# hku-mars/ImMesh

Measured on AMD Instinct MI355X. Metric: scans/sec (reg+mesh), 100k-pt scan into 10M-voxel map, higher is better.
Workload: dtype f64

## Files before the change

immesh_amd/csrc/c_api.cpp:

```cpp
#include "host_ctx.hpp"
#include "imu_host.hpp"
#include <cmath>
#include <new>

#define RP_ABORTED 1
static thread_local std::string g_create_error;
thread_local KProf* g_kprof = nullptr;



extern "C" {

void immesh_default_config(immesh_config* c) {
    std::memset(c, 0, sizeof(*c));
    c->voxel_size = 0.5; c->max_layer = 2;
    for (int i = 0; i < 5; i++) c->layer_init[i] = 5;
    c->max_points_size = 100; c->planer_threshold = 0.01; c->dept_err = 0.02; c->beam_err = 0.05; c->calib_laser = 0;
    c->sigma_num = 3.0; c->max_iter = 4;
    c->extR[0] = c->extR[4] = c->extR[8] = 1.0;
    c->extT[0] = 0.04165; c->extT[1] = 0.02326; c->extT[2] = -0.0284;
    c->mesh_min_spacing = 0.1; c->mesh_voxel = 0.4; c->mesh_region = 10.0; c->mesh_append_budget = 10000;
}

const char* immesh_create_error(void) { return g_create_error.c_str(); }
const char* immesh_last_error(immesh_ctx* c) { return c ? c->err.c_str() : "null ctx"; }

static int alloc_all(immesh_ctx* c) {
    const immesh_config& g = c->cfg;
    RegMapDev& m = c->map;
    const int64_t cap_roots = g.cap_root_voxels > 0 ? g.cap_root_voxels : (1 << 20);
    const int64_t cap_nodes = g.cap_nodes > 0 ? g.cap_nodes : cap_roots + cap_roots / 2;
    const int64_t cap_chunks = g.cap_point_chunks > 0 ? g.cap_point_chunks : cap_nodes * 2;
    const int64_t cap_ext = g.max_points_size > IM_INLINE_CHUNKS * IM_CHUNK_PTS ? std::max<int64_t>(1024, cap_nodes / 4) : std::max<int64_t>(1024, cap_nodes / 64);
    const int64_t hcap = np2(cap_roots * 2);
    if (cap_nodes > 0x7fffffff || cap_chunks > 0x7fffffff || hcap > 0xffffffffLL) { c->err = "capacity too large for 32-bit indices"; return IMMESH_E_INVAL; }
    int rc;
#define A(ptr, n) if ((rc = c->dalloc(&(ptr), (size_t)(n)))) return rc
    A(m.htab, hcap); A(m.slot_head, hcap);
    m.hmask = (uint64_t)hcap - 1;
    A(m.nodes, cap_nodes);
    const int64_t cap_leaf = std::max<int64_t>(4096, cap_nodes / 2);
    A(m.leaf_chunks, cap_leaf * 16); m.cap_leaf_chunks = (int32_t)cap_leaf;
    A(m.chunk_data, cap_chunks * IM_CHUNK_PTS * IM_PT_DOUBLES); A(m.ext_tables, cap_ext * IM_EXT_CHUNKS);
    A(m.counters, 16); A(m.free_ready, cap_chunks); A(m.free_pending, cap_chunks);
    m.cap_nodes = (int32_t)cap_nodes; m.cap_chunks = (int32_t)cap_chunks; m.cap_ext = (int32_t)cap_ext;
    m.max_layer = g.max_layer; m.max_points_size = g.max_points_size;
    for (int i = 0; i < 5; i++) m.init_size[i] = g.layer_init[i];
    m.planer_threshold = (float)g.planer_threshold;
    m.voxel_size_f = (float)g.voxel_size;
    m.voxel_size_d = g.voxel_size;
    m.shard_rank = g.shard_world > 1 ? g.shard_rank : 0; m.shard_world = g.shard_world > 1 ? g.shard_world : 1;
    m.shard_brick_log2 = g.shard_brick_log2 > 0 ? g.shard_brick_log2 : 5;
    m.shard_scheme = g.shard_scheme == 1 ? 1 : 0;
    HIPCHK(c, hipMemsetAsync(m.counters, 0, 16 * sizeof(int32_t), c->stream));
    HIPCHK(c, hipMemsetAsync(m.htab, 0xFF, hcap * sizeof(HashEnt), c->stream));
    HIPCHK(c, hipMemsetAsync(m.slot_head, 0, hcap * sizeof(unsigned long long), c->stream));
    m.upd_seq = 0;
    A(c->d_stats, STATS_WORDS);
    if (c->knobs.debug) { A(c->reg_dbg, REG_DBG_WORDS); HIPCHK(c, hipMemsetAsync(c->reg_dbg, 0, (size_t)REG_DBG_WORDS * 8, c->stream)); }
    HIPCHK(c, hipMemsetAsync(c->d_stats, 0, STATS_WORDS * sizeof(int64_t), c->stream));

    const int64_t ns = g.cap_scan_points > 0 ? g.cap_scan_points : 600000;
    c->cap_scan = ns;
    A(c->d_pts_down, ns * 3); A(c->d_pts_raw, ns * 4);
    A(c->d_partials, ((ns + 63) / 64) * RES_NR); A(c->d_out48, RES_NV); A(c->d_done, 4);
    HIPCHK(c, hipMemsetAsync(c->d_done, 0, 16, c->stream));
    A(c->d_match, ns); A(c->d_mnode, ns); A(c->d_dis, ns); A(c->d_rinv, ns); A(c->d_normal, ns * 3);
    A(c->d_ptdata, ns * IM_PT_DOUBLES);
    A(c->d_key_a, ns); A(c->d_key_b, ns); A(c->d_idx_a, ns); A(c->d_idx_b, ns); A(c->d_idx_c, ns);
    A(c->d_slot, ns); A(c->d_slot_s, ns); A(c->d_seg_start, ns); A(c->d_nseg, 16); A(c->d_ds_out, ns * 3);
    c->sort_temp_bytes = std::max({sort_pairs_u64_temp_bytes((int)ns), sort_pairs_u32_temp_bytes((int)ns), exclusive_sum_temp_bytes((int)ns)}) + 256;
    { char* t; A(t, c->sort_temp_bytes); c->d_sort_temp = t; }
    A(c->p_key_a, ns); A(c->p_key_b, ns); A(c->p_idx_a, ns); A(c->p_idx_b, ns); A(c->p_idx_c, ns); A(c->p_seg, ns); A(c->p_nseg, 16); A(c->p_slot, ns); A(c->p_slot_s, ns); A(c->p_pool4, ns * 4);
    { char* t; A(t, c->sort_temp_bytes); c->p_sort_temp = t; }
    {
        unsigned long long cap = 1024; while (cap < 2ull * (unsigned long long)ns) cap <<= 1;
        char* t; A(t, cap * 16); c->p_htab = t; c->p_htab_cap = cap;
        launch_ds_table_reset(c->stream, t, cap);
        if ((rc = c->pinned(&c->h_ds_dyn, &c->d_ds_dyn, 1)) || (rc = c->pinned(&c->h_ds_info, &c->d_ds_info, 16))) return rc;
        HIPCHK(c, hipMemsetAsync(c->p_nseg, 0, 16 * sizeof(int32_t), c->stream));
    }
    {
        m.split_general = c->knobs.split_general >= 0 ? c->knobs.split_general : (g.max_layer >= 3 ? 1 : 0);
        A(m.sub_order, ns); A(m.sub_items, 2 * ns);
        HIPCHK(c, hipMemsetAsync(m.sub_items, 0, (size_t)2 * ns * sizeof(unsigned long long), c->stream));
    }
    A(c->d_dump_count, 2);
    A(c->d_touched, 2 * ns + 16);
    A(c->d_regstate, 1);
    A(c->d_epi, 8);
    HIPCHK(c, hipMemsetAsync(c->d_epi, 0, 32, c->stream));
    for (int q = 0; q < 2; q++) { A(c->d_rp_slots[q], RP_SLOT_DOUBLES); launch_fill_u64(c->stream, (unsigned long long*)c->d_rp_slots[q], RP_SLOT_SENTINEL, RP_SLOT_DOUBLES); }
    HIPCHK(c, hipMemsetAsync(c->d_regstate, 0, sizeof(RegState), c->stream));
    A(c->d_und_in, ns * 5); A(c->d_und_out, ns * 4); A(c->d_und_tab, 64 * 23 + 24);
#undef A
    if ((rc = c->pinned(&c->h_out48, &c->d_out48_host, RES_NV)) || (rc = c->pinned(&c->h_reg_out, &c->d_reg_out_host, REG_OUT_DOUBLES)) ||
        (rc = c->pinned(&c->h_epi_flag, &c->d_epi_flag_host, 8)) || (rc = c->pinned(&c->h_counters, &c->d_counters_host, 16))) return rc;
    return 0;
}


immesh_ctx* immesh_create(const immesh_config* cfg) {
    g_create_error.clear();
    if (!cfg) { g_create_error = "null config"; return nullptr; }
    int ndev = 0;
    hipError_t e = hipGetDeviceCount(&ndev);
    if (e != hipSuccess || ndev <= 0) {
        g_create_error = std::string("no usable HIP device (") + (e != hipSuccess ? hipGetErrorString(e) : "count 0") + "); the hot path has no CPU fallback";
        return nullptr;
    }
    if (cfg->device < 0 || cfg->device >= ndev) { g_create_error = "device ordinal out of range"; return nullptr; }
    if (cfg->max_layer < 0 || cfg->max_layer > 4 || cfg->voxel_size <= 0 || cfg->max_iter < 1) { g_create_error = "invalid config"; return nullptr; }
    if (cfg->shard_world > 1 && (cfg->shard_rank < 0 || cfg->shard_rank >= cfg->shard_world || cfg->shard_brick_log2 < 0 || cfg->shard_brick_log2 > 16)) { g_create_error = "invalid shard configuration"; return nullptr; }
    immesh_ctx* c = new (std::nothrow) immesh_ctx();
    if (!c) { g_create_error = "out of host memory"; return nullptr; }
    c->cfg = *cfg;
    c->knobs = Knobs::from_env(MESH_NPAR);
    std::memset(&c->cnt, 0, sizeof(c->cnt));
    int prio_greatest = 0;
    if (hipSetDevice(cfg->device) == hipSuccess) (void)hipDeviceGetStreamPriorityRange(&c->prio_least, &prio_greatest);
    if (c->knobs.no_priority) prio_greatest = c->prio_least = 0;
    if (c->knobs.make_stream(&c->stream, prio_greatest, false) != hipSuccess) {
        g_create_error = "hipSetDevice/hipStreamCreate failed"; delete c; return nullptr;
    }
    for (auto& ev : c->ev) (void)hipEventCreate(&ev);
    if (c->knobs.make_stream(&c->stream_pre, 0, true) != hipSuccess || hipEventCreateWithFlags(&c->ev_inputs_free, hipEventDisableTiming) != hipSuccess ||
        hipEventRecord(c->ev_inputs_free, c->stream) != hipSuccess || !(c->ev_inputs_cur = c->ev_inputs_free)) {
        g_create_error = "hipStreamCreate/hipEventCreate failed"; immesh_destroy(c); return nullptr;
    }
    { const double s = std::sin((double)(float)cfg->beam_err * 0.017453293); c->dvar_beam = s * s; }
    { const double s = std::sin((double)(float)0.01 * 0.017453293); c->dvar_calib = s * s; }
    {
        const int resident = residual_persistent_resident_blocks(cfg->device);
        c->rp_max_blocks = c->knobs.rp_blocks ? c->knobs.rp_blocks : std::max(1, resident / 2 - 1);
    }
    int rc = alloc_all(c);
    if (!rc) rc = mesh_alloc(c);
    if (!rc && hipStreamSynchronize(c->stream) != hipSuccess) { rc = IMMESH_E_HIP; c->err = "initialisation kernels failed"; }
    if (rc) { g_create_error = c->err; immesh_destroy(c); return nullptr; }
// ... 645 lines not shown
```

immesh_amd/csrc/reg_kernels.hip:

```cpp
#include <algorithm>
#include <cstdlib>
#include "regmap.hpp"
#include "kernels.hpp"
#include "prof.hpp"

using namespace imd;

struct PlaneRegs { double n[3], c[3], pv[21]; float d, radius; };
struct BestMatch { int node; int layer; double prob; bool ok; PlaneRegs P; };

IMD double plane_sigma(const double* pv, const double* J) {
    double tmp[6];
#pragma unroll
    for (int c = 0; c < 6; c++) {
        double s = 0;
#pragma unroll
        for (int r = 0; r < 6; r++) s += J[r] * pv[(r <= c) ? sym21_index(r, c) : sym21_index(c, r)];
        tmp[c] = s;
    }
    double sig = 0;
#pragma unroll
    for (int c = 0; c < 6; c++) sig += tmp[c] * J[c];
    return sig;
}
// ... 1074 lines not shown
        else v = e < 36 ? rs->p11inv[e] : (e < 108 ? rs->tmat[e - 36] : (e < 132 ? rs->st[e - 108] : (e < 156 ? rs->prior[e - 132] : (e < 160 ? rs->tot[e - 156] : (double)rs->rematch))));
        L[400 + e] = v;
    }
    if (a.it == 0) {
        for (int e = lane; e < 108; e += 64) { if (e < 36) rs->p11inv[e] = a.mat[e]; else rs->tmat[e - 36] = a.mat[e]; }
        if (lane < 24) rs->prior[lane] = a.prior[lane];
        const unsigned long long* src = (const unsigned long long*)&a.sp;
        unsigned long long* dst = (unsigned long long*)&rs->sp;
        for (int e = lane; e < (int)(sizeof(ScanParams) / 8); e += 64) dst[e] = src[e];
    }
    __syncthreads();
    if (lane == 0) { L[400 + 156] += L[64 + RES_PLANE_TESTS]; L[400 + 157] += L[64 + RES_EXTRA_PROBE]; L[400 + 159] += L[64 + RES_N_MATCH]; }
    __syncthreads();
    ekf_step_wave(rs, L + 400, a.mat, L + 64 + RES_HTH, L + 64 + RES_HTZ, L[64 + RES_N_MATCH], L[64 + RES_SUM_DIS], L + 128, lane, a.it, a.max_iter, a.sp.extR, reg_out, ticket);
}

IMD float4 transform_value(const double* extR, const double* extT, const double* R, const double* t, const float4 v) {
    const double p[3] = {(double)v.x, (double)v.y, (double)v.z};
    double pi[3], pw[3];
    m3_vec(extR, p, pi);
    pi[0] += extT[0]; pi[1] += extT[1]; pi[2] += extT[2];
    m3_vec(R, pi, pw);
    return make_float4((float)(pw[0] + t[0]), (float)(pw[1] + t[1]), (float)(pw[2] + t[2]), v.w);
}
IMD void transform_point(const double* extR, const double* extT, const double* R, const double* t, const float4* __restrict__ raw, float4* __restrict__ world, const int i) {
    world[i] = transform_value(extR, extT, R, t, raw[i]);
}
IMD void point_var_point(const RegMapDev& m, const ScanParams& sp, const float* __restrict__ pts, const int i, const int stride, const int mode,
                         double* __restrict__ pt_data, unsigned long long* __restrict__ sort_key, uint32_t* __restrict__ slot_out, int32_t* __restrict__ pt_next,
                         const unsigned long long hint_key, const unsigned int hint_slot, const int hint_root) {
    const double p[3] = {(double)pts[(size_t)i * stride + 0], (double)pts[(size_t)i * stride + 1], (double)pts[(size_t)i * stride + 2]};
    double pimu[3], pwd[3];
    m3_vec(sp.extR, p, pimu);
    pimu[0] += sp.extT[0]; pimu[1] += sp.extT[1]; pimu[2] += sp.extT[2];
    m3_vec(sp.R, pimu, pwd);
    pwd[0] += sp.t[0]; pwd[1] += sp.t[1]; pwd[2] += sp.t[2];
    const double pw[3] = {(double)(float)pwd[0], (double)(float)pwd[1], (double)(float)pwd[2]};
    double bcov[9], cm[9], a[9];
    if (mode == 0) {
        double pz[3] = {p[0], p[1], p[2]};
        if (pz[2] == 0) pz[2] = 0.001;
        calc_body_var(pz, sp.dept_err, sp.dvar_beam, bcov);
        double pimu_z[3];
        m3_vec(sp.extR, pz, pimu_z);
        pimu_z[0] += sp.extT[0]; pimu_z[1] += sp.extT[1]; pimu_z[2] += sp.extT[2];
        skew(pimu_z, cm);
        m3_sandwich(sp.RextR, bcov, a);
    } else {
        double pl[3] = {p[0], p[1], p[2]};
        calc_body_var(pl, sp.dept_err, sp.dvar_beam, bcov);
        skew(pl, cm);
        m3_sandwich(sp.R, bcov, a);
    }
    double nc[9], tmp[9], b[9], var[9];
#pragma unroll
    for (int k = 0; k < 9; k++) nc[k] = -cm[k];
    m3_mul(nc, sp.rot_var, tmp);
    m3_mul_bt(tmp, nc, b);
#pragma unroll
    for (int k = 0; k < 9; k++) var[k] = (a[k] + b[k]) + sp.t_var[k];
    double* o = pt_data + (size_t)i * IM_PT_DOUBLES;
    o[0] = pw[0]; o[1] = pw[1]; o[2] = pw[2];
    o[3] = var[0]; o[4] = var[1]; o[5] = var[2]; o[6] = var[4]; o[7] = var[5]; o[8] = var[8];
    const double key = sqrt(var[0] * var[0] + var[4] * var[4] + var[8] * var[8]);
    sort_key[i] = (unsigned long long)__double_as_longlong(key);
    int64_t kx[3];
#pragma unroll
    for (int j = 0; j < 3; j++) kx[j] = key_axis(pw[j] / (double)m.voxel_size_f);
    const uint64_t pk = pack_key(kx[0], kx[1], kx[2]);
    if (m.shard_world > 1 && !shard_keeps(m, kx[0], kx[1], kx[2])) { slot_out[i] = 0xFFFFFFFFu; return; }
    bool created = false;
    const bool hinted = hint_root >= 0 && pk == hint_key;
    const int64_t slot = hinted ? (int64_t)hint_slot : hash_find_or_insert(m, pk, &created);
    if (slot < 0) { m.counters[5] = 5; slot_out[i] = 0xFFFFFFFFu; return; }
    if (created) {
        const float vs = m.voxel_size_f;
        const double c[3] = {(0.5 + (double)kx[0]) * (double)vs, (0.5 + (double)kx[1]) * (double)vs, (0.5 + (double)kx[2]) * (double)vs};
        const int node = node_alloc(m, 0, c, vs / 4, pk, 0);
        m.htab[slot].root = node;
        atomicAdd(&m.counters[6], 1);
    }
    slot_out[i] = (uint32_t)slot;
    if (pt_next) {
        const unsigned long long mine = ((unsigned long long)(unsigned int)m.upd_seq << 32) | (unsigned int)i;
        const unsigned long long old = atomicExch(&m.slot_head[slot], mine);
        const bool first = (unsigned int)(old >> 32) != (unsigned int)m.upd_seq;
        const unsigned long long fm = __ballot(first);
        if (first) {
            pt_next[i] = -1;
            const int lane = (int)(threadIdx.x & 63), leader = __builtin_ctzll(fm);
            int base = 0;
            if (lane == leader) base = atomicAdd(&m.counters[7], (int)__popcll(fm));
            base = __shfl(base, leader, 64);
            const int k = base + (int)__popcll(fm & ((1ull << lane) - 1ull));
            m.touched[2 * (size_t)k] = (uint32_t)slot; m.touched[2 * (size_t)k + 1] = hinted ? (uint32_t)hint_root : (uint32_t)m.htab[slot].root;
        }
        else pt_next[i] = (int)(unsigned int)(old & 0xFFFFFFFFull);
    }
}

__global__ __launch_bounds__(256) void point_var_kernel(RegMapDev m, ScanParams sp, const ScanParams* __restrict__ spd, const float* __restrict__ pts, int n, int stride, int mode,
                                                         double* __restrict__ pt_data, unsigned long long* __restrict__ sort_key, uint32_t* __restrict__ slot_out,
                                                         int32_t* __restrict__ pt_next, const float4* __restrict__ raw, float4* __restrict__ world, int n_raw, int nb_pv) {
    if ((int)blockIdx.x >= nb_pv) {
        const int i = ((int)blockIdx.x - nb_pv) * 256 + threadIdx.x;
        if (i >= n_raw) return;
        const ScanParams* q = spd ? spd : &sp;
        double R[9], t[3];
#pragma unroll
        for (int k = 0; k < 9; k++) R[k] = q->R[k];
#pragma unroll
        for (int k = 0; k < 3; k++) t[k] = q->t[k];
        transform_point(sp.extR, sp.extT, R, t, raw, world, i);
        return;
    }
    const int i = blockIdx.x * blockDim.x + threadIdx.x;
    if (i >= n) return;
    if (spd) {
#pragma unroll
        for (int k = 0; k < 9; k++) { sp.R[k] = spd->R[k]; sp.RextR[k] = spd->RextR[k]; sp.rot_var[k] = spd->rot_var[k]; sp.t_var[k] = spd->t_var[k]; }
#pragma unroll
        for (int k = 0; k < 3; k++) sp.t[k] = spd->t[k];
    }
    point_var_point(m, sp, pts, i, stride, mode, pt_data, sort_key, slot_out, pt_next);
}

__global__ void segment_heads_kernel(const uint32_t* __restrict__ sorted_slot, int n, int32_t* __restrict__ seg_start, int32_t* __restrict__ nseg) {
    const int i = blockIdx.x * blockDim.x + threadIdx.x;
    if (i >= n) return;
    if (sorted_slot[i] == 0xFFFFFFFFu) return;
    if (i == 0 || sorted_slot[i - 1] != sorted_slot[i]) seg_start[atomicAdd(nseg, 1)] = i;
}

struct WaveCtx { int lane; int64_t* stats; int root; bool shared = false; };

struct PlaneFit { double c[3], ev[3], U[9]; int imin, imax; bool planar; };
IMD double sel3(const int i, const double a, const double b, const double c) { return i == 0 ? a : (i == 1 ? b : c); }

template <class FE>
IMD void fit_eigen(FE&& for_each_point, const int n, const float planer_threshold, PlaneFit& f) {
    double s[9];
#pragma unroll
    for (int k = 0; k < 9; k++) s[k] = 0;
    for_each_point([&](const double* q) __attribute__((always_inline)) {
        const double x = q[0], y = q[1], z = q[2];
        s[0] += x; s[1] += y; s[2] += z;
        s[3] += x * x; s[4] += x * y; s[5] += x * z; s[6] += y * y; s[7] += y * z; s[8] += z * z;
    });
#pragma unroll
    for (int k = 0; k < 9; k++) s[k] = wave_sum_fast(s[k]);
    const double dn = (double)n;
    f.c[0] = s[0] / dn; f.c[1] = s[1] / dn; f.c[2] = s[2] / dn;
    double cov[9];
    cov[0] = s[3] / dn - f.c[0] * f.c[0]; cov[1] = s[4] / dn - f.c[0] * f.c[1]; cov[2] = s[5] / dn - f.c[0] * f.c[2];
    cov[3] = cov[1];                      cov[4] = s[6] / dn - f.c[1] * f.c[1]; cov[5] = s[7] / dn - f.c[1] * f.c[2];
    cov[6] = cov[2];                      cov[7] = cov[5];                      cov[8] = s[8] / dn - f.c[2] * f.c[2];
    sym3_eigen_jacobi_fast(cov, f.ev, f.U);
    const double e0 = f.ev[0], e1 = f.ev[1], e2 = f.ev[2];
    int imin = 0, imax = 0;
    double emin = e0, emax = e0;
    if (e1 < emin) { imin = 1; emin = e1; }
    if (e2 < emin) { imin = 2; emin = e2; }
    if (e1 > emax) { imax = 1; emax = e1; }
    if (e2 > emax) { imax = 2; emax = e2; }
    f.imin = imin; f.imax = imax;
    f.planar = emin < (double)planer_threshold;
}

template <class FE>
IMD void fit_plane_var(FE&& for_each_point, const int n, const PlaneFit& f, double* pv) {
#pragma clang fp contract(fast)
    const int imin = f.imin, m1 = imin == 0 ? 1 : 0, m2 = imin == 2 ? 1 : 2;
    double um1[3], um2[3], umin[3];
#pragma unroll
    for (int r = 0; r < 3; r++) {
        const double u0 = f.U[r * 3 + 0], u1 = f.U[r * 3 + 1], u2 = f.U[r * 3 + 2];
        um1[r] = sel3(m1, u0, u1, u2);
        um2[r] = sel3(m2, u0, u1, u2);
        umin[r] = sel3(imin, u0, u1, u2);
    }
// ... 450 lines not shown
            if (last_refit_n) { (void)wave_init_plane(m, node, last_refit_n, wq); last_refit_n = 0; }
            if (w.lane == 0) { nd.flags = nd.flags & ~NF_UPDATE_EN; node_free_points(m, node); nd.newpts = 0; }
            __builtin_amdgcn_fence(__ATOMIC_RELEASE, "workgroup");
            npts = 0; newp = 0;
            j++;
            if (w.lane == 0 && w.stats && n_ref) { atomicAdd((unsigned long long*)&w.stats[0], (unsigned long long)n_ref); atomicAdd((unsigned long long*)&w.stats[1], (unsigned long long)n_ref_pts); }
            return j;
        }
    }
    write_counts();
    if (last_refit_n) (void)wave_init_plane(m, node, last_refit_n, wq);
    if (w.lane == 0 && w.stats && n_ref) { atomicAdd((unsigned long long*)&w.stats[0], (unsigned long long)n_ref); atomicAdd((unsigned long long*)&w.stats[1], (unsigned long long)n_ref_pts); }
    return j;
}

__global__ __launch_bounds__(256) void replay_kernel(RegMapDev m, const uint32_t* __restrict__ sorted_slot, const int32_t* __restrict__ sorted_idx,
                                                      const double* __restrict__ pt_data, int n, const int32_t* __restrict__ seg_start,
                                                      const int32_t* __restrict__ nseg, int mode, int64_t* stats) {
    __shared__ int stacks[4][48];
    const int wv = threadIdx.x >> 6;
    const int seg = blockIdx.x * 4 + wv;
    if (seg >= *nseg) return;
    WaveCtx w; w.lane = threadIdx.x & 63; w.stats = stats;
    const int start = seg_start[seg];
    const uint32_t slot = sorted_slot[start];
    const int root = m.htab[slot].root;
    if (root < 0) return;
    w.root = root;
    if (mode == 0) {
        for (int j = start; j < n && sorted_slot[j] == slot; j++)
            wave_update_point(m, root, pt_data + (size_t)sorted_idx[j] * IM_PT_DOUBLES, stacks[wv], w);
    } else {
        int cnt = m.nodes[root].npts;
        for (int j = start; j < n && sorted_slot[j] == slot; j++) {
            if (!wave_push_point(m, root, cnt, pt_data + (size_t)sorted_idx[j] * IM_PT_DOUBLES, w)) return;
            cnt++;
        }
        if (w.lane == 0) { m.nodes[root].npts = cnt; m.nodes[root].newpts = cnt; }
        __builtin_amdgcn_fence(__ATOMIC_RELEASE, "workgroup");
        if (cnt > m.init_size[0]) wave_init_octo_tree(m, root, stacks[wv], w);
    }
}

#define RL_CAP 64
#define DBG_FUSED_OFF 64
#define DBG_FUSED_RECS 16384
#define DBG_RES_OFF (DBG_FUSED_OFF + DBG_FUSED_RECS * 8)
static_assert(DBG_RES_OFF + 8 * 512 * 8 == REG_DBG_WORDS, "the IMMESH_DEBUG buffer (kernels.hpp) holds the counters and both trace areas");
#define RF_PTS 128
__global__ __launch_bounds__(256, 3) void replay_fused_kernel(RegMapDev m, const int32_t* __restrict__ pt_next, const unsigned long long* __restrict__ sort_key,
                                                            const double* __restrict__ pt_data, int64_t* stats, uint32_t* __restrict__ general_list,
                                                            unsigned long long* __restrict__ dbg, unsigned long long* flag_dev, unsigned long long* flag_host,
                                                            unsigned long long flag_seq) {
    if (flag_dev && blockIdx.x == 0 && threadIdx.x == 0) {
        __hip_atomic_store(flag_dev, flag_seq, __ATOMIC_RELAXED, __HIP_MEMORY_SCOPE_AGENT);
        __hip_atomic_store(flag_host, flag_seq, __ATOMIC_RELAXED, __HIP_MEMORY_SCOPE_SYSTEM);
    }
    __shared__ unsigned long long skey[4][RL_CAP];
    __shared__ int sidx[4][RL_CAP];
    __shared__ int order[4][RL_CAP];
    __builtin_amdgcn_s_setprio(REG_UPD_PRIO);
    const int wv = threadIdx.x >> 6, lane = threadIdx.x & 63;
    const int t_first = blockIdx.x * 4 + wv, t_stride = gridDim.x * 4;
    uint32_t slot_first = m.touched[2 * (size_t)t_first];
    int root_first = (int)m.touched[2 * (size_t)t_first + 1];
    const int n_touched = m.counters[7];
#define FDBG(k) do { if (dbg) { const unsigned long long _t = __builtin_readcyclecounter(); if (tr) ((unsigned int*)tr)[4 + (k)] = (unsigned int)(_t - tprev); tprev = _t; } } while (0)
#define FEND(state, nref) do { if (tr) { tr[1] = __builtin_amdgcn_s_memrealtime(); tr[7] = (unsigned long long)((unsigned)cnt | ((unsigned)(nref) << 8) | ((unsigned)(state) << 16)); } } while (0)
    auto process = [&](const int t, const uint32_t slot, int root) __attribute__((always_inline)) {
    unsigned long long* const tr = (dbg && lane == 0 && t < DBG_FUSED_RECS) ? dbg + DBG_FUSED_OFF + (size_t)t * 8 : nullptr;
    unsigned long long tprev = dbg ? __builtin_readcyclecounter() : 0;
    if (tr) { tr[0] = __builtin_amdgcn_s_memrealtime(); tr[2] = tr[3] = tr[4] = tr[5] = tr[6] = tr[7] = 0; }
    if (root < 0) root = m.htab[slot].root;
    if (root < 0) return;
    FDBG(0);
    NodeRec& nd = m.nodes[root];
    const int flags = nd.flags, layer = nd.layer;
    const int npts = nd.npts, newp = nd.newpts;
    if (dbg) { asm volatile("s_waitcnt vmcnt(0)" ::: "memory"); FDBG(1); }
    int chunks[IM_INLINE_CHUNKS];
#pragma unroll
    for (int k = 0; k < IM_INLINE_CHUNKS; k++) chunks[k] = nd.chunks[k];
    if (dbg) { asm volatile("s_waitcnt vmcnt(0)" ::: "memory"); FDBG(2); }
    int cnt = 0;
    int ihead = (int)(unsigned int)(m.slot_head[slot] & 0xFFFFFFFFull);
    if (dbg) { asm volatile("s_waitcnt vmcnt(0)" ::: "memory"); FDBG(3); }
    for (int i = ihead; i >= 0; i = pt_next[i]) {
        if (cnt < RL_CAP && lane == 0) { skey[wv][cnt] = sort_key[i]; sidx[wv][cnt] = i; }
        cnt++;
    }
    FDBG(4);
    const int want = NF_INIT | NF_PLANE | NF_UPDATE_EN;
    if (layer == 0 && (flags & want) == (NF_INIT | NF_PLANE)) { FEND(1, 0); return; }
    const int ntot = npts + cnt;
    bool hand_over = cnt > RL_CAP || (flags & want) != want || layer != 0 || newp > 5 || ntot > RF_PTS || ntot >= m.max_points_size;
    if (!hand_over) {
        __builtin_amdgcn_fence(__ATOMIC_RELEASE, "workgroup");
        __builtin_amdgcn_wave_barrier();
        __builtin_amdgcn_fence(__ATOMIC_ACQUIRE, "workgroup");
        for (int e = lane; e < cnt; e += 64) {
            const unsigned long long k = skey[wv][e];
            const int id = sidx[wv][e];
            int rank = 0;
            for (int f = 0; f < cnt; f++) { const unsigned long long kf = skey[wv][f]; rank += (kf < k || (kf == k && sidx[wv][f] < id)) ? 1 : 0; }
            order[wv][rank] = id;
        }
        __builtin_amdgcn_fence(__ATOMIC_RELEASE, "workgroup");
        __builtin_amdgcn_wave_barrier();
        __builtin_amdgcn_fence(__ATOMIC_ACQUIRE, "workgroup");
        FDBG(5);
        auto chunk_of = [&](int ci) { int c = chunks[0];
#pragma unroll
            for (int k = 1; k < IM_INLINE_CHUNKS; k++) { const int ck = chunks[k]; c = (ci == k) ? ck : c; }
            return c; };
        const int n_ref = (newp + cnt) / 6;
        double P0[9], P1[9];
#pragma unroll
        for (int k = 0; k < 9; k++) { P0[k] = 0; P1[k] = 0; }
        {
            const int q0 = lane, q1 = lane + 64;
            const double* s0 = nullptr; const double* s1 = nullptr;
            if (q0 < ntot && (q0 >= npts || n_ref > 0))
                s0 = q0 < npts ? m.chunk_data + ((size_t)chunk_of(q0 >> 4) * IM_CHUNK_PTS + (q0 & 15)) * IM_PT_DOUBLES : pt_data + (size_t)order[wv][q0 - npts] * IM_PT_DOUBLES;
            if (q1 < ntot && (q1 >= npts || n_ref > 0))
                s1 = q1 < npts ? m.chunk_data + ((size_t)chunk_of(q1 >> 4) * IM_CHUNK_PTS + (q1 & 15)) * IM_PT_DOUBLES : pt_data + (size_t)order[wv][q1 - npts] * IM_PT_DOUBLES;
            if (s0) {
#pragma unroll
                for (int k = 0; k < 9; k++) P0[k] = s0[k]; }
            if (s1) {
#pragma unroll
                for (int k = 0; k < 9; k++) P1[k] = s1[k]; }
        }
        if (dbg) asm volatile("s_waitcnt vmcnt(0)" ::: "memory");
        FDBG(6);
        PlaneFit fit;
        long long n_ref_pts = 0;
        int n_last = 0;
        for (int r = 0; r < n_ref && !hand_over; r++) {
            const int nr = npts + 6 * (r + 1) - newp;
            n_ref_pts += nr;
            auto fe = [&](auto&& fn) __attribute__((always_inline)) { if (lane < nr) fn(P0); if (lane + 64 < nr) fn(P1); };
            if (r + 1 < n_ref) {
                double s1[3] = {0, 0, 0}, s2[3] = {0, 0, 0};
                fe([&](const double* q) __attribute__((always_inline)) {
#pragma unroll
                    for (int a = 0; a < 3; a++) { s1[a] += q[a]; s2[a] += q[a] * q[a]; } });
#pragma unroll
                for (int a = 0; a < 3; a++) { s1[a] = wave_sum_fast(s1[a]); s2[a] = wave_sum_fast(s2[a]); }
                const double dn = (double)nr;
                double vmin = 1e300, mag = 0;
#pragma unroll
                for (int a = 0; a < 3; a++) { const double mu = s1[a] / dn; const double v = s2[a] / dn - mu * mu; vmin = fmin(vmin, v); mag += s2[a] / dn; }
                if (vmin + (1e-7 + 1e-12 * mag) < (double)m.planer_threshold) continue;
            }
            fit_eigen(fe, nr, m.planer_threshold, fit);
            if (!fit.planar) hand_over = true;
            n_last = nr;
        }
        FDBG(7);
        if (!hand_over) {
            const int c_first = (npts + IM_CHUNK_PTS - 1) >> 4, c_last = (ntot - 1) >> 4;
            if (cnt > 0 && c_first <= c_last) {
                int c = 0;
                const bool need = lane >= c_first && lane <= c_last && lane < IM_INLINE_CHUNKS && chunk_of(lane) < 0;
                if (need) c = alloc_chunk(m);
                if (__ballot(need && c < 0)) return;
#pragma unroll
                for (int k = 0; k < IM_INLINE_CHUNKS; k++) { const int ck = __shfl(c, k, 64); const int nk = __shfl(need ? 1 : 0, k, 64); if (nk) chunks[k] = ck; }
            }
            {
                const int q0 = lane, q1 = lane + 64;
                if (q0 >= npts && q0 < ntot) { double* d = m.chunk_data + ((size_t)chunk_of(q0 >> 4) * IM_CHUNK_PTS + (q0 & 15)) * IM_PT_DOUBLES;
#pragma unroll
                    for (int k = 0; k < 9; k++) d[k] = P0[k]; }
                if (q1 >= npts && q1 < ntot) { double* d = m.chunk_data + ((size_t)chunk_of(q1 >> 4) * IM_CHUNK_PTS + (q1 & 15)) * IM_PT_DOUBLES;
#pragma unroll
                    for (int k = 0; k < 9; k++) d[k] = P1[k]; }
            }
            if (lane == 0) {
                nd.npts = ntot; nd.newpts = (newp + cnt) % 6;
#pragma unroll
                for (int k = 0; k < IM_INLINE_CHUNKS; k++) nd.chunks[k] = chunks[k];
                if (n_ref) { int64_t* sh = stats + 16 + (size_t)(t & 63) * 16; atomicAdd((unsigned long long*)&sh[0], (unsigned long long)n_ref); atomicAdd((unsigned long long*)&sh[1], (unsigned long long)n_ref_pts); }
            }
            FDBG(8);
            if (n_ref > 0) {
                double pv[21];
                auto fe = [&](auto&& fn) __attribute__((always_inline)) { if (lane < n_last) fn(P0); if (lane + 64 < n_last) fn(P1); };
                fit_plane_var(fe, n_last, fit, pv);
                fit_store(nd, fit, pv, lane);
            }
            FDBG(9);
            FEND(2, n_ref);
            return;
        }
    }
    if (lane == 0) general_list[atomicAdd(&m.counters[10], 1)] = slot;
    FEND(3, 0);
    };
    for (int t = t_first; t < n_touched; t += t_stride) {
        if (t != t_first) { slot_first = m.touched[2 * (size_t)t]; root_first = (int)m.touched[2 * (size_t)t + 1]; }
        process(t, slot_first, root_first);
    }
#undef FDBG
#undef FEND
}

__device__ bool replay_split_root(const RegMapDev& m, const int root, const int* order, const int cnt, const double* __restrict__ pt_data, const WaveCtx& w);
__device__ bool replay_split_leaves(const RegMapDev& m, const int root, const int* order, const int cnt, const double* __restrict__ pt_data, const WaveCtx& w, int* s_key, int* s_first);
__global__ __launch_bounds__(256) void replay_list_kernel(RegMapDev m, const int32_t* __restrict__ pt_next, const unsigned long long* __restrict__ sort_key,
                                                           const double* __restrict__ pt_data, int64_t* stats, int32_t* __restrict__ big_idx, int32_t* __restrict__ big_order,
                                                           unsigned long long* __restrict__ dbg, const uint32_t* __restrict__ work, const int32_t* __restrict__ n_work) {
    __shared__ unsigned long long skey[4][RL_CAP];
    __shared__ int sidx[4][RL_CAP];
    __shared__ int order[4][RL_CAP];
    __shared__ int stacks[4][48];
    __builtin_amdgcn_s_setprio(REG_UPD_PRIO);
    const int wv = threadIdx.x >> 6;
    const int nw = *n_work;
    WaveCtx w; w.lane = threadIdx.x & 63; w.stats = stats;
    for (int t = blockIdx.x * 4 + wv; t < nw; t += gridDim.x * 4) {
        const uint32_t slot = work[t];
        const int root = m.htab[slot].root;
        if (root < 0) continue;
        w.root = root;
        const unsigned long long tdbg0 = dbg ? __builtin_readcyclecounter() : 0;
        __builtin_amdgcn_wave_barrier();
        int cnt = 0;
        for (int i = (int)(unsigned int)(m.slot_head[slot] & 0xFFFFFFFFull); i >= 0; i = pt_next[i]) {
            if (cnt < RL_CAP && w.lane == 0) { skey[wv][cnt] = sort_key[i]; sidx[wv][cnt] = i; }
            cnt++;
        }
        if (cnt > RL_CAP) {
            int base = 0;
            if (w.lane == 0) base = atomicAdd(&m.counters[9], cnt);
            base = __shfl(base, 0, 64);
            if (w.lane == 0) { int k = 0; for (int i = (int)(unsigned int)(m.slot_head[slot] & 0xFFFFFFFFull); i >= 0; i = pt_next[i]) big_idx[base + k++] = i; }
            __builtin_amdgcn_fence(__ATOMIC_RELEASE, "agent");
            __builtin_amdgcn_wave_barrier();
            __builtin_amdgcn_fence(__ATOMIC_ACQUIRE, "agent");
            for (int e = w.lane; e < cnt; e += 64) {
                const int id = big_idx[base + e];
                const unsigned long long k = sort_key[id];
                int rank = 0;
                for (int f = 0; f < cnt; f++) { const int idf = big_idx[base + f]; const unsigned long long kf = sort_key[idf]; rank += (kf < k || (kf == k && idf < id)) ? 1 : 0; }
                big_order[base + rank] = id;
            }
            __builtin_amdgcn_fence(__ATOMIC_RELEASE, "agent");
            __builtin_amdgcn_wave_barrier();
            __builtin_amdgcn_fence(__ATOMIC_ACQUIRE, "agent");
            if (replay_split_root(m, root, big_order + base, cnt, pt_data, w)) continue;
            int jb = wave_replay_planar_root(m, root, big_order + base, cnt, pt_data, w);
            if (jb == 0) jb = wave_replay_planar_node(m, root, big_order + base, cnt, pt_data, w);
            for (int j = jb; j < cnt; j++) wave_update_point(m, root, pt_data + (size_t)big_order[base + j] * IM_PT_DOUBLES, stacks[wv], w);
            continue;
        }
        __builtin_amdgcn_fence(__ATOMIC_RELEASE, "workgroup");
        __builtin_amdgcn_wave_barrier();
        __builtin_amdgcn_fence(__ATOMIC_ACQUIRE, "workgroup");
        for (int e = w.lane; e < cnt; e += 64) {
            const unsigned long long k = skey[wv][e];
            const int id = sidx[wv][e];
            int rank = 0;
            for (int f = 0; f < cnt; f++) { const unsigned long long kf = skey[wv][f]; rank += (kf < k || (kf == k && sidx[wv][f] < id)) ? 1 : 0; }
            order[wv][rank] = id;
        }
        __builtin_amdgcn_fence(__ATOMIC_RELEASE, "workgroup");
        __builtin_amdgcn_wave_barrier();
        __builtin_amdgcn_fence(__ATOMIC_ACQUIRE, "workgroup");
        if (replay_split_leaves(m, root, order[wv], cnt, pt_data, w, (int*)skey[wv], sidx[wv])) continue;
        if (replay_split_root(m, root, order[wv], cnt, pt_data, w)) continue;
        const unsigned long long tdbg1 = dbg ? __builtin_readcyclecounter() : 0;
        int jf = wave_replay_planar_root(m, root, order[wv], cnt, pt_data, w);
        if (jf == 0) jf = wave_replay_planar_node(m, root, order[wv], cnt, pt_data, w);
        for (int j = jf; j < cnt; j++) wave_update_point(m, root, pt_data + (size_t)order[wv][j] * IM_PT_DOUBLES, stacks[wv], w);
        if (dbg && w.lane == 0) {
            const unsigned long long t2 = __builtin_readcyclecounter();
            atomicMax(&dbg[jf == cnt ? 8 : 9], ((t2 - tdbg0) << 16) | (unsigned long long)cnt);
            atomicAdd(&dbg[jf == cnt ? 10 : 11], t2 - tdbg1);
            atomicAdd(&dbg[jf == cnt ? 12 : 13], 1ull);
            atomicAdd(&dbg[14], tdbg1 - tdbg0);
        }
    }
}

#define SPLIT_MISSING 0x40000000
__device__ __noinline__ bool replay_split_leaves(const RegMapDev& m, const int root, const int* order, const int cnt, const double* __restrict__ pt_data, const WaveCtx& w, int* s_key, int* s_first) {
    const NodeRec& nr = m.nodes[root];
    const int flags = nr.flags;
    if (!m.split_general || cnt < 2 || cnt > RL_CAP || !(flags & NF_INIT) || (flags & NF_PLANE) || nr.layer >= m.max_layer || m.cap_nodes >= (1 << 26)) return false;
    if (w.lane == 0 && nr.npts != 0) node_free_points(m, root);
    const int lane = w.lane;
    int key = -1;
    if (lane < cnt) {
        const double* q = pt_data + (size_t)order[lane] * IM_PT_DOUBLES;
        const double qx = q[0], qy = q[1], qz = q[2];
        int nd = root;
        for (int depth = 0; depth < 8; depth++) {
            const NodeRec& r = m.nodes[nd];
            const int f = r.flags, layer = r.layer, npts = r.npts;
            if (!((f & NF_INIT) && !(f & NF_PLANE) && layer < m.max_layer && (npts == 0 || nd == root))) { key = nd; break; }
            const int oct = 4 * (qx > r.center[0] ? 1 : 0) + 2 * (qy > r.center[1] ? 1 : 0) + (qz > r.center[2] ? 1 : 0);
            const int child = r.child[oct];
            if (child < 0) { key = nd | (oct << 26) | SPLIT_MISSING; break; }
            nd = child;
        }
        if (key < 0) key = nd;
    }
    if (lane < cnt) s_key[lane] = key;
    __builtin_amdgcn_fence(__ATOMIC_RELEASE, "workgroup");
    __builtin_amdgcn_wave_barrier();
    __builtin_amdgcn_fence(__ATOMIC_ACQUIRE, "workgroup");
    int first = lane, rank = 0, size = 0;
    if (lane < cnt) {
        first = -1;
        for (int f = 0; f < cnt; f++) {
            const bool same = s_key[f] == key;
            if (same && first < 0) first = f;
            if (same && f < lane) rank++;
            if (same) size++;
        }
        s_first[lane] = first;
    }
    __builtin_amdgcn_fence(__ATOMIC_RELEASE, "workgroup");
    __builtin_amdgcn_wave_barrier();
    __builtin_amdgcn_fence(__ATOMIC_ACQUIRE, "workgroup");
    int before = 0;
    if (lane < cnt) for (int f = 0; f < cnt; f++) before += s_first[f] < first ? 1 : 0;
    const bool leader = lane < cnt && first == lane;
    const unsigned long long lm = __ballot(leader);
    const int n_items = (int)__popcll(lm);
    int seg = 0, item0 = 0;
    if (lane == 0) { seg = atomicAdd(&m.counters[11], cnt); item0 = atomicAdd(&m.counters[12], n_items); }
    seg = __shfl(seg, 0, 64); item0 = __shfl(item0, 0, 64);
    if (lane < cnt) m.sub_order[seg + before + rank] = order[lane];
    if (leader) {
        const int it = item0 + (int)__popcll(lm & ((1ull << lane) - 1ull));
        const int start = (key & SPLIT_MISSING) ? (key & ((1 << 26) - 1)) : key;
        m.sub_items[2 * (size_t)it] = (unsigned long long)(unsigned int)start | ((unsigned long long)(unsigned int)root << 32);
        m.sub_items[2 * (size_t)it + 1] = (unsigned long long)(unsigned int)(seg + before) | ((unsigned long long)(unsigned int)size << 32);
    }
    return true;
}
__device__ bool replay_split_root(const RegMapDev& m, const int root, const int* order, const int cnt, const double* __restrict__ pt_data, const WaveCtx& w) {
    const NodeRec& nr = m.nodes[root];
    const int flags = nr.flags;
    if (!m.split_general || cnt < 8 || !(flags & NF_INIT) || (flags & NF_PLANE) || nr.layer >= m.max_layer) return false;
    if (w.lane == 0 && nr.npts != 0) node_free_points(m, root);
// ... 190 lines not shown
```

immesh_amd/csrc/regmap.hpp:

```cpp
#pragma once
#include "dev_math.hpp"

#define IM_CHUNK_PTS 16
#define IM_PT_DOUBLES 9
#define IM_INLINE_CHUNKS 8
#define IM_EXT_CHUNKS 2048
#define IM_LEAF_SLOTS 15
#define IM_G_MAX_POINTS 1000

#define NF_INIT 1
#define NF_PLANE 2
#define NF_UPDATE_EN 4

struct alignas(64) NodeRec {
    int32_t child[8];
    int32_t flags, layer, npts, newpts;
    float quarter, d, radius, min_eig;
    double center[3];
    double p_center[3];
    double p_normal[3];
    double p_var[21];
    int32_t chunks[IM_INLINE_CHUNKS];
    int32_t ext, path;
    unsigned long long key;
    int32_t leaf_head;
    int32_t lock;
    unsigned long long pad[3];
};
static_assert(sizeof(NodeRec) == 384, "NodeRec layout");

struct HashEnt { unsigned long long key; int32_t root; int32_t pad; };

struct RegMapDev {
    HashEnt* htab;
    uint64_t hmask;
    NodeRec* nodes;
    double* chunk_data;
    int32_t* ext_tables;
    int32_t* counters;
    int32_t* free_ready;
    int32_t* free_pending;
    int32_t* leaf_chunks;
    int32_t cap_leaf_chunks;
    unsigned long long* slot_head;
    uint32_t* touched;
    int32_t split_general;
    int32_t* sub_order;
    unsigned long long* sub_items;
    int32_t upd_seq;
    int32_t shard_rank, shard_world, shard_brick_log2, shard_scheme;
    int32_t cap_nodes, cap_chunks, cap_ext;
    int32_t max_layer, max_points_size, init_size[5];
    float planer_threshold;
    float voxel_size_f;
    double voxel_size_d;
};

namespace imd {

IMD int sym21_index(int r, int c) {
    return r * 6 - (r * (r - 1)) / 2 + (c - r);
}

IMHD int brick_owner(int scheme, int world, int64_t bx, int64_t by, int64_t bz, uint64_t packed) {
    if (scheme == 1 || world % 3 == 0 || world % 5 == 0) return (int)(hash64(packed) % (uint64_t)world);
    const int64_t c = (bx + 3 * by + 5 * bz) % (int64_t)world;
    return (int)(c < 0 ? c + world : c);
}
IMD int shard_owner(const RegMapDev& m, int64_t kx, int64_t ky, int64_t kz) {
    const int b = m.shard_brick_log2;
    return brick_owner(m.shard_scheme, m.shard_world, kx >> b, ky >> b, kz >> b, pack_key(kx >> b, ky >> b, kz >> b));
}
IMD bool shard_keeps(const RegMapDev& m, int64_t kx, int64_t ky, int64_t kz) {
    if (shard_owner(m, kx, ky, kz) == m.shard_rank) return true;
    const int64_t msk = ((int64_t)1 << m.shard_brick_log2) - 1;
    const int64_t lx = kx & msk, ly = ky & msk, lz = kz & msk;
    if (lx != 0 && lx != msk && ly != 0 && ly != msk && lz != 0 && lz != msk) return false;
    for (int dx = -1; dx <= 1; dx++)
        for (int dy = -1; dy <= 1; dy++)
            for (int dz = -1; dz <= 1; dz++)
                if ((dx | dy | dz) != 0 && shard_owner(m, kx + dx, ky + dy, kz + dz) == m.shard_rank) return true;
    return false;
}

IMD int64_t hash_find(const RegMapDev& m, uint64_t key) {
    uint64_t h = hash64(key) & m.hmask;
    for (int probe = 0; probe < 4096; probe++) {
        const unsigned long long k = m.htab[h].key;
        if (k == key) return (int64_t)h;
        if (k == IM_KEY_EMPTY) return -1;
        h = (h + 1) & m.hmask;
    }
    return -1;
}
IMD int64_t hash_find_or_insert(const RegMapDev& m, uint64_t key, bool* created) {
    uint64_t h = hash64(key) & m.hmask;
    *created = false;
    for (int probe = 0; probe < 4096; probe++) {
        unsigned long long k = m.htab[h].key;
        if (k == key) return (int64_t)h;
        if (k == IM_KEY_EMPTY) {
            const unsigned long long prev = atomicCAS(&m.htab[h].key, (unsigned long long)IM_KEY_EMPTY, (unsigned long long)key);
            if (prev == IM_KEY_EMPTY) { *created = true; return (int64_t)h; }
            if (prev == key) return (int64_t)h;
        }
        h = (h + 1) & m.hmask;
    }
    return -1;
}

IMD int alloc_chunk(const RegMapDev& m) {
    if (__hip_atomic_load(&m.counters[2], __ATOMIC_RELAXED, __HIP_MEMORY_SCOPE_AGENT) > 0) {
        int i = atomicSub(&m.counters[2], 1) - 1;
        if (i >= 0) return m.free_ready[i];
        atomicAdd(&m.counters[2], 1);
    }
    const int c = atomicAdd(&m.counters[1], 1);
    if (c >= m.cap_chunks) { m.counters[5] = 1; return -1; }
    return c;
}
IMD void free_chunk(const RegMapDev& m, int c) {
    if (c < 0) return;
    const int i = atomicAdd(&m.counters[3], 1);
    m.free_pending[i] = c;
}
IMD int node_chunk_id(const RegMapDev& m, int node, int ci) {
    if (ci < IM_INLINE_CHUNKS) return m.nodes[node].chunks[ci];
    const int e = m.nodes[node].ext;
    return m.ext_tables[(size_t)e * IM_EXT_CHUNKS + (ci - IM_INLINE_CHUNKS)];
}
IMD double* node_point_ptr(const RegMapDev& m, int node, int i) {
    const int c = node_chunk_id(m, node, i / IM_CHUNK_PTS);
// ... 95 lines not shown
```

Measured before the change: 6038.

## Store first per-voxel point indices in slot records to avoid linked-list chasing

The per-slot linked list of incoming points is replaced by a counter plus a fixed 8-word record per hash slot. The first seven point indices go directly into the record and only overflow points go into the pt_next chain. The update kernels now load the record lane-parallel instead of walking a serial dependent chain from lane 0. This adds a per-slot record array the size of the hash table and two atomics per point, one fetch_max and one fetch_add.

```diff
diff --git a/immesh_amd/csrc/c_api.cpp b/immesh_amd/csrc/c_api.cpp
--- a/immesh_amd/csrc/c_api.cpp
+++ b/immesh_amd/csrc/c_api.cpp
@@ -36,7 +36,7 @@
     if (cap_nodes > 0x7fffffff || cap_chunks > 0x7fffffff || hcap > 0xffffffffLL) { c->err = "capacity too large for 32-bit indices"; return IMMESH_E_INVAL; }
     int rc;
 #define A(ptr, n) if ((rc = c->dalloc(&(ptr), (size_t)(n)))) return rc
-    A(m.htab, hcap); A(m.slot_head, hcap);
+    A(m.htab, hcap); A(m.slot_head, hcap); A(m.slot_rec, hcap * IM_SLOT_REC);
     m.hmask = (uint64_t)hcap - 1;
     A(m.nodes, cap_nodes);
     const int64_t cap_leaf = std::max<int64_t>(4096, cap_nodes / 2);
@@ -55,6 +55,7 @@
     HIPCHK(c, hipMemsetAsync(m.counters, 0, 16 * sizeof(int32_t), c->stream));
     HIPCHK(c, hipMemsetAsync(m.htab, 0xFF, hcap * sizeof(HashEnt), c->stream));
     HIPCHK(c, hipMemsetAsync(m.slot_head, 0, hcap * sizeof(unsigned long long), c->stream));
+    HIPCHK(c, hipMemsetAsync(m.slot_rec, 0xFF, hcap * IM_SLOT_REC * sizeof(int32_t), c->stream));
     m.upd_seq = 0;
     A(c->d_stats, STATS_WORDS);
     if (c->knobs.debug) { A(c->reg_dbg, REG_DBG_WORDS); HIPCHK(c, hipMemsetAsync(c->reg_dbg, 0, (size_t)REG_DBG_WORDS * 8, c->stream)); }
diff --git a/immesh_amd/csrc/reg_kernels.hip b/immesh_amd/csrc/reg_kernels.hip
--- a/immesh_amd/csrc/reg_kernels.hip
+++ b/immesh_amd/csrc/reg_kernels.hip
@@ -1180,12 +1180,18 @@
     }
     slot_out[i] = (uint32_t)slot;
     if (pt_next) {
-        const unsigned long long mine = ((unsigned long long)(unsigned int)m.upd_seq << 32) | (unsigned int)i;
-        const unsigned long long old = atomicExch(&m.slot_head[slot], mine);
-        const bool first = (unsigned int)(old >> 32) != (unsigned int)m.upd_seq;
+        const unsigned long long stamp = (unsigned long long)(unsigned int)m.upd_seq << 32;
+        __hip_atomic_fetch_max(&m.slot_head[slot], stamp, __ATOMIC_RELAXED, __HIP_MEMORY_SCOPE_AGENT);
+        const unsigned long long old = __hip_atomic_fetch_add(&m.slot_head[slot], 1ull, __ATOMIC_RELAXED, __HIP_MEMORY_SCOPE_AGENT);
+        const unsigned int pos = (unsigned int)(old & 0xFFFFFFFFull);
+        const bool first = pos == 0;
+        int32_t* const rec = m.slot_rec + (size_t)slot * IM_SLOT_REC;
+        if (pos < IM_SLOT_VP) rec[pos] = i;
+        else {
+            pt_next[i] = __hip_atomic_exchange(&rec[IM_SLOT_VP], i, __ATOMIC_RELAXED, __HIP_MEMORY_SCOPE_AGENT);
+        }
         const unsigned long long fm = __ballot(first);
         if (first) {
-            pt_next[i] = -1;
             const int lane = (int)(threadIdx.x & 63), leader = __builtin_ctzll(fm);
             int base = 0;
             if (lane == leader) base = atomicAdd(&m.counters[7], (int)__popcll(fm));
@@ -1193,7 +1199,6 @@
             const int k = base + (int)__popcll(fm & ((1ull << lane) - 1ull));
             m.touched[2 * (size_t)k] = (uint32_t)slot; m.touched[2 * (size_t)k + 1] = hinted ? (uint32_t)hint_root : (uint32_t)m.htab[slot].root;
         }
-        else pt_next[i] = (int)(unsigned int)(old & 0xFFFFFFFFull);
     }
 }
 
@@ -1810,28 +1815,33 @@
 #pragma unroll
     for (int k = 0; k < IM_INLINE_CHUNKS; k++) chunks[k] = nd.chunks[k];
     if (dbg) { asm volatile("s_waitcnt vmcnt(0)" ::: "memory"); FDBG(2); }
-    int cnt = 0;
-    int ihead = (int)(unsigned int)(m.slot_head[slot] & 0xFFFFFFFFull);
+    const int cnt = (int)(unsigned int)(m.slot_head[slot] & 0xFFFFFFFFull);
+    int ll = lane;
+    asm volatile("" : "+v"(ll));
+    const int rec_word = ll < IM_SLOT_REC ? m.slot_rec[(size_t)slot * IM_SLOT_REC + ll] : -1;
     if (dbg) { asm volatile("s_waitcnt vmcnt(0)" ::: "memory"); FDBG(3); }
-    for (int i = ihead; i >= 0; i = pt_next[i]) {
-        if (cnt < RL_CAP && lane == 0) { skey[wv][cnt] = sort_key[i]; sidx[wv][cnt] = i; }
-        cnt++;
-    }
-    FDBG(4);
     const int want = NF_INIT | NF_PLANE | NF_UPDATE_EN;
-    if (layer == 0 && (flags & want) == (NF_INIT | NF_PLANE)) { FEND(1, 0); return; }
+    if (layer == 0 && (flags & want) == (NF_INIT | NF_PLANE)) { FDBG(4); FEND(1, 0); return; }
     const int ntot = npts + cnt;
     bool hand_over = cnt > RL_CAP || (flags & want) != want || layer != 0 || newp > 5 || ntot > RF_PTS || ntot >= m.max_points_size;
     if (!hand_over) {
+        int id = rec_word;
+        if (cnt > IM_SLOT_VP) {
+            int i = __shfl(rec_word, IM_SLOT_VP, 64);
+            for (int k = IM_SLOT_VP; k < cnt; k++) { if (ll == k) id = i; if (k + 1 < cnt) i = pt_next[i]; }
+        }
+        if (ll < cnt) { skey[wv][ll] = sort_key[id]; sidx[wv][ll] = id; }
+        if (dbg) asm volatile("s_waitcnt vmcnt(0)" ::: "memory");
+        FDBG(4);
         __builtin_amdgcn_fence(__ATOMIC_RELEASE, "workgroup");
         __builtin_amdgcn_wave_barrier();
         __builtin_amdgcn_fence(__ATOMIC_ACQUIRE, "workgroup");
         for (int e = lane; e < cnt; e += 64) {
             const unsigned long long k = skey[wv][e];
-            const int id = sidx[wv][e];
+            const int ide = sidx[wv][e];
             int rank = 0;
-            for (int f = 0; f < cnt; f++) { const unsigned long long kf = skey[wv][f]; rank += (kf < k || (kf == k && sidx[wv][f] < id)) ? 1 : 0; }
-            order[wv][rank] = id;
+            for (int f = 0; f < cnt; f++) { const unsigned long long kf = skey[wv][f]; rank += (kf < k || (kf == k && sidx[wv][f] < ide)) ? 1 : 0; }
+            order[wv][rank] = ide;
         }
         __builtin_amdgcn_fence(__ATOMIC_RELEASE, "workgroup");
         __builtin_amdgcn_wave_barrier();
@@ -1949,21 +1959,24 @@
     WaveCtx w; w.lane = threadIdx.x & 63; w.stats = stats;
     for (int t = blockIdx.x * 4 + wv; t < nw; t += gridDim.x * 4) {
         const uint32_t slot = work[t];
+        const int cnt = (int)(unsigned int)(m.slot_head[slot] & 0xFFFFFFFFull);
+        int ll = w.lane;
+        asm volatile("" : "+v"(ll));
+        const int rec_word = ll < IM_SLOT_REC ? m.slot_rec[(size_t)slot * IM_SLOT_REC + ll] : -1;
         const int root = m.htab[slot].root;
         if (root < 0) continue;
         w.root = root;
         const unsigned long long tdbg0 = dbg ? __builtin_readcyclecounter() : 0;
         __builtin_amdgcn_wave_barrier();
-        int cnt = 0;
-        for (int i = (int)(unsigned int)(m.slot_head[slot] & 0xFFFFFFFFull); i >= 0; i = pt_next[i]) {
-            if (cnt < RL_CAP && w.lane == 0) { skey[wv][cnt] = sort_key[i]; sidx[wv][cnt] = i; }
-            cnt++;
-        }
         if (cnt > RL_CAP) {
             int base = 0;
             if (w.lane == 0) base = atomicAdd(&m.counters[9], cnt);
             base = __shfl(base, 0, 64);
-            if (w.lane == 0) { int k = 0; for (int i = (int)(unsigned int)(m.slot_head[slot] & 0xFFFFFFFFull); i >= 0; i = pt_next[i]) big_idx[base + k++] = i; }
+            if (ll < IM_SLOT_VP) big_idx[base + ll] = rec_word;
+            {
+                int i = __shfl(rec_word, IM_SLOT_VP, 64);
+                for (int k = IM_SLOT_VP; k < cnt; k++) { if (w.lane == 0) big_idx[base + k] = i; if (k + 1 < cnt) i = pt_next[i]; }
+            }
             __builtin_amdgcn_fence(__ATOMIC_RELEASE, "agent");
             __builtin_amdgcn_wave_barrier();
             __builtin_amdgcn_fence(__ATOMIC_ACQUIRE, "agent");
@@ -1983,15 +1996,21 @@
             for (int j = jb; j < cnt; j++) wave_update_point(m, root, pt_data + (size_t)big_order[base + j] * IM_PT_DOUBLES, stacks[wv], w);
             continue;
         }
+        int id = rec_word;
+        if (cnt > IM_SLOT_VP) {
+            int i = __shfl(rec_word, IM_SLOT_VP, 64);
+            for (int k = IM_SLOT_VP; k < cnt; k++) { if (ll == k) id = i; if (k + 1 < cnt) i = pt_next[i]; }
+        }
+        if (ll < cnt) { skey[wv][ll] = sort_key[id]; sidx[wv][ll] = id; }
         __builtin_amdgcn_fence(__ATOMIC_RELEASE, "workgroup");
         __builtin_amdgcn_wave_barrier();
         __builtin_amdgcn_fence(__ATOMIC_ACQUIRE, "workgroup");
         for (int e = w.lane; e < cnt; e += 64) {
             const unsigned long long k = skey[wv][e];
-            const int id = sidx[wv][e];
+            const int ide = sidx[wv][e];
             int rank = 0;
-            for (int f = 0; f < cnt; f++) { const unsigned long long kf = skey[wv][f]; rank += (kf < k || (kf == k && sidx[wv][f] < id)) ? 1 : 0; }
-            order[wv][rank] = id;
+            for (int f = 0; f < cnt; f++) { const unsigned long long kf = skey[wv][f]; rank += (kf < k || (kf == k && sidx[wv][f] < ide)) ? 1 : 0; }
+            order[wv][rank] = ide;
         }
         __builtin_amdgcn_fence(__ATOMIC_RELEASE, "workgroup");
         __builtin_amdgcn_wave_barrier();
diff --git a/immesh_amd/csrc/regmap.hpp b/immesh_amd/csrc/regmap.hpp
--- a/immesh_amd/csrc/regmap.hpp
+++ b/immesh_amd/csrc/regmap.hpp
@@ -7,6 +7,8 @@
 #define IM_EXT_CHUNKS 2048
 #define IM_LEAF_SLOTS 15
 #define IM_G_MAX_POINTS 1000
+#define IM_SLOT_VP 7
+#define IM_SLOT_REC 8
 
 #define NF_INIT 1
 #define NF_PLANE 2
@@ -42,12 +44,13 @@
     int32_t* free_pending;
     int32_t* leaf_chunks;
     int32_t cap_leaf_chunks;
+    int32_t upd_seq;
     unsigned long long* slot_head;
+    int32_t* slot_rec;
     uint32_t* touched;
     int32_t split_general;
     int32_t* sub_order;
     unsigned long long* sub_items;
-    int32_t upd_seq;
     int32_t shard_rank, shard_world, shard_brick_log2, shard_scheme;
     int32_t cap_nodes, cap_chunks, cap_ext;
     int32_t max_layer, max_points_size, init_size[5];
```

Result: no change. 6023 (-0.3%).
